# lofcz/Infidex

Hardware: AMD Instinct MI355X
Metric: queries/sec, 10M-doc corpus, top-k=20 (whole hot path, index resident in HBM) (higher is better)
Workload: dtype f32; 1 GPU; BASELINE config 4: 10000000 docs, vocab 1000000, 1 field(s), 1000-query batches, 2-3-word queries 30% fuzzed, depth 500, top-20; docs=10000000, batch=1000, top_k=20, coverage_depth=500, sessions_in_flight=4, parallelism=single GPU

## Files before the change

infidex_amd/csrc/infidex_hip.hip:

```cpp
#include <type_traits>
#include <cstring>
#include <hip/hip_runtime.h>
#include <stdint.h>
#include <string.h>
#include <stdio.h>
#include <string>
#include <vector>
#include <unordered_map>
#include <algorithm>
#include <map>
#include <mutex>
#include <chrono>
#include <thread>
#include <dlfcn.h>
#include <rccl/rccl.h>
#include "../../include/infidex_hip.h"
#include "unicode_tables.h"

#define WAVE 64
#define FILT_MAXCOL 64

static thread_local std::string g_err;
static int32_t fail(int32_t code, const char* fmt, const char* a = "") {
    char buf[512]; snprintf(buf, sizeof buf, fmt, a); g_err = buf; return code;
// ... 91 lines not shown
    uint64_t a = lo, b = hi;
    while (a < b) { uint64_t m = (a + b) >> 1; if ((int64_t)(packed ? (int32_t)((uint32_t)postDoc[m] >> 8) : postDoc[m]) < target) a = m + 1; else b = m; }
    skipTbl[(uint64_t)s * per + r] = (uint32_t)(a - lo);
}

__global__ void k_doc_norm(const float* docLen, float* norm, int n, float bDivAvg) {
    int i = blockIdx.x * blockDim.x + threadIdx.x;
    if (i >= n) return;
    const float k1 = 1.2f, minDl = 1.f - 0.75f;
    float t1 = bDivAvg * docLen[i];
    float t2 = minDl + t1;
    norm[i] = k1 * t2;
}

struct DevTerm {
    uint64_t begin, end;
    float idf;
    uint32_t skip;
    uint8_t role, rank, isVirtual, pad;
    uint16_t refIdx, pad2;
};
struct DevQuery {
    uint32_t termOff, numTerms;
    int32_t mode, prefixSet, depth, nAnd;
    uint32_t refOff, numRef;
};
struct SelRule {
    int32_t mode;
    int32_t cutoffRank;
    uint32_t classMask;
    int32_t depth;
    uint32_t total;
    uint32_t pad;
};

template <class Tp> __device__ __forceinline__ Tp rfl(Tp v) { return v; }
__device__ __forceinline__ int rfl_i(int v) { return __builtin_amdgcn_readfirstlane(v); }
__device__ __forceinline__ uint64_t rfl_u64(uint64_t v) {
    uint32_t lo = __builtin_amdgcn_readfirstlane((uint32_t)v), hi = __builtin_amdgcn_readfirstlane((uint32_t)(v >> 32));
    return ((uint64_t)hi << 32) | lo;
}

__device__ __forceinline__ int32_t post_doc(int32_t v, int packed) { return packed ? (int32_t)((uint32_t)v >> 8) : v; }
__device__ __forceinline__ uint64_t lower_bound_post(const int32_t* a, uint64_t lo, uint64_t hi, int32_t target, int packed) {
    while (lo < hi) { uint64_t m = (lo + hi) >> 1; if (post_doc(a[m], packed) < target) lo = m + 1; else hi = m; }
    return lo;
}
__device__ __forceinline__ uint64_t lower_bound_i32(const int32_t* a, uint64_t lo, uint64_t hi, int32_t target) {
    while (lo < hi) { uint64_t m = (lo + hi) >> 1; if (a[m] < target) lo = m + 1; else hi = m; }
    return lo;
}

#include "stage1.hip.inc"
#include "stage1_sparse.hip.inc"
#include "exact1.hip.inc"
#include "exact3.hip.inc"
#include "exactsh.hip.inc"
#include "stage2.hip.inc"

__host__ __device__ static inline SelRule make_rule0(const infx_query& Q, const uint32_t* c) {
    SelRule r{}; r.mode = Q.mode; r.depth = Q.depth; r.cutoffRank = 127; r.classMask = 0xFFFFFFFFu;
    const long k = Q.depth;
    if (Q.mode == INFX_MODE_AND) {
        unsigned long long t0 = 0, t1 = 0;
        for (int i = 0; i < 16; i++) { if (i & 1) t0 += c[i]; if (i & 2) t1 += c[i]; }
        if ((long)t0 >= k * 2) { r.classMask = 1; return r; }
        unsigned long long g = t0; uint32_t gmask = 1;
        if (Q.n_and >= 3 && (long)t0 < k * 3) { g = t1; gmask = 2 | 1; }
        if ((long)g < k * 5) {
            if (Q.df_s1 <= 0) { r.classMask = gmask; return r; }
            if ((long)Q.df_s1 >= k * 10 || Q.df_s2 <= 0) { r.classMask = 4 | gmask; return r; }
            r.classMask = 4 | 8 | gmask; return r;
        }
        r.classMask = gmask; return r;
    }
    if (Q.mode == INFX_MODE_DISJ) {
        int nElig = Q.n_and; bool hasSel = false; long local = 0; int cutoff = -1;
        int nRanks = 0; for (int i = 127; i >= 0; i--) if (c[i]) { nRanks = i + 1; break; }
        int totalRanks = nRanks > Q.df_s1 ? nRanks : Q.df_s1;
        for (int i = 0; i < totalRanks; i++) {
            bool lowq = i >= nElig;
            if (totalRanks > 1 && lowq && hasSel) continue;
            cutoff = i; local += c[i];
            if (!lowq && local > 0) hasSel = true;
            if (local >= k * 100) break;
        }
        r.cutoffRank = cutoff; return r;
    }
    return r;
}

__host__ __device__ static inline SelRule make_rule(const infx_query& Q, const uint32_t* c) {
    SelRule r = make_rule0(Q, c);
    unsigned long long tot = 0;
    if (Q.mode == INFX_MODE_AND) { for (int i = 0; i < 16; i++) if (i & r.classMask) tot += c[i]; }
    else if (Q.mode == INFX_MODE_DISJ) { for (int i = 0; i <= r.cutoffRank && i < 128; i++) tot += c[i]; tot += 128;  }
    else tot = c[1];
    r.total = (uint32_t)(tot < 0xFFFFFFFFull ? tot : 0xFFFFFFFFull); r.pad = 0;
    return r;
}

#include "fused.hip.inc"
#include "lookup.hip.inc"
#include "filter.hip.inc"
#include "browse.hip.inc"
#include "facets_filtered.hip.inc"
// ... 304 lines not shown
    if (!bytes) return INFX_OK;
    if (!is_device_ptr(src)) return up(s, dst, src, bytes);
    HIPCHK(hipMemcpyAsync(dst, src, bytes, hipMemcpyDeviceToDevice, s->st)); s->unsynced = true;
    return INFX_OK;
}
static int32_t downx(infx_stream* s, void* dst, const void* srcDev, size_t bytes) {
    if (!bytes) return INFX_OK;
    if (!is_device_ptr(dst)) return down(s, dst, srcDev, bytes);
    HIPCHK(hipMemcpyAsync(dst, srcDev, bytes, hipMemcpyDeviceToDevice, s->st)); s->unsynced = true;
    return INFX_OK;
}
struct PlanStream {
    infx_stream* s; bool on;
    explicit PlanStream(infx_stream* x) : s(x), on(x->stPlan != nullptr) { if (on) s->st = s->stPlan; }
    int32_t leave() {
        if (!on) return INFX_OK;
        on = false; s->st = s->stMain;
        HIPCHK(hipEventRecord(s->evPlan, s->stPlan));
        HIPCHK(hipStreamWaitEvent(s->stMain, s->evPlan, 0));
        return INFX_OK;
    }
    ~PlanStream() { if (on) s->st = s->stMain; }
};
#define UPX(dst, src, n) do { int32_t rc_ = upx(s, (dst), (src), (n)); if (rc_) return rc_; } while (0)
#define DOWNX(dst, src, n) do { int32_t rc_ = downx(s, (dst), (src), (n)); if (rc_) return rc_; } while (0)
#define UP(dst, src, n) do { int32_t rc_ = up(s, (dst), (src), (n)); if (rc_) return rc_; } while (0)
#define DOWN(dst, src, n) do { int32_t rc_ = down(s, (dst), (src), (n)); if (rc_) return rc_; } while (0)
#define SYNC() do { int32_t rc_ = stream_sync(s); if (rc_) return rc_; } while (0)
static int32_t table_upload(infx_stream* s, const ProgTable& T, void** buf, size_t* cap) {
    const size_t total = T.blob_bytes();
    { int32_t rc_ = grow(s, buf, cap, total); if (rc_) return rc_; }
    std::vector<uint8_t> H(total, 0);
    T.put_blob(H.data(), (const char*)*buf);
    return up(s, *buf, H.data(), total);
}
#define COLS_COVER_CORPUS "a column holds fewer rows than the corpus has documents%s"
#define COLS_COVER_COUNTED "a column holds fewer rows than the counted documents%s"
static int32_t columns_cover(const infx_index* ix, int64_t n, const char* msg, int col = -1) {
    for (int c = std::max(col, 0); c < (col < 0 ? FILT_MAXCOL : col + 1); c++)
        if (ix->colCodes[c] && (uint64_t)ix->colDocs[c] < (uint64_t)std::max<int64_t>(n, 0)) return fail(INFX_EINVAL, msg);
    return INFX_OK;
}
static DevColumns dev_columns(const infx_index* ix) { DevColumns cols; for (int c = 0; c < FILT_MAXCOL; c++) cols.codes[c] = ix->colCodes[c]; return cols; }
static hipError_t lds_limit(const void* fn, int device, size_t lds) {
    if (lds <= 64 * 1024) return hipSuccess;
    static std::mutex mu; static std::map<std::pair<int, const void*>, size_t> mark;
    std::lock_guard<std::mutex> lk(mu);
    size_t& hw = mark[{device, fn}];
    if (lds > hw) { const hipError_t e = hipFuncSetAttribute(fn, hipFuncAttributeMaxDynamicSharedMemorySize, (int)lds); if (e != hipSuccess) return e; hw = lds; }
    return hipSuccess;
}

template <int R> static void launch_union(infx_stream* s, uint32_t nv, const uint32_t* dBeg, const uint32_t* dEnd, const int32_t* dMembers, uint32_t* dRangeCount,
                                            const unsigned long long* dBase, int32_t* outDocs) {
    uint64_t blocks = (uint64_t)nv * s->ix->d.nRanges;
    k_union<R><<<dim3((unsigned)blocks), dim3(WAVE), 0, s->st>>>(dev_index(s), dBeg, dEnd, dMembers, nv, dRangeCount, dBase, outDocs);
}
static void launch_union_any(infx_stream* s, uint32_t nv, const uint32_t* dBeg, const uint32_t* dEnd, const int32_t* dMembers, uint32_t* dRangeCount,
                             const unsigned long long* dBase, int32_t* outDocs) {
    switch (s->ix->d.R) {
        case 512: launch_union<512>(s, nv, dBeg, dEnd, dMembers, dRangeCount, dBase, outDocs); break;
        case 1024: launch_union<1024>(s, nv, dBeg, dEnd, dMembers, dRangeCount, dBase, outDocs); break;
        case 2048: launch_union<2048>(s, nv, dBeg, dEnd, dMembers, dRangeCount, dBase, outDocs); break;
        case 4096: launch_union<4096>(s, nv, dBeg, dEnd, dMembers, dRangeCount, dBase, outDocs); break;
        case 8192: launch_union<8192>(s, nv, dBeg, dEnd, dMembers, dRangeCount, dBase, outDocs); break;
        default: launch_union<16384>(s, nv, dBeg, dEnd, dMembers, dRangeCount, dBase, outDocs); break;
    }
}
static bool exact_enabled(const infx_index* ix) { static const bool v = [] { const char* e = getenv("INFX_EXACT"); return !(e && e[0] == '0'); }(); return v && !(ix->cfg.flags & INFX_CFG_NO_EXACT_REPLAY); }
static Arena make_arena(infx_stream* s) {
    return Arena{s->arDoc, s->arScore, s->arCls, s->arMask, s->arExc, (const unsigned long long*)s->dBlockOut, (uint32_t*)s->dBlockOutHi,
                 (uint32_t*)s->dCounts, s->dOverflow, (unsigned long long*)s->dQBytes, (uint32_t*)((unsigned long long*)s->dQBytes + s->lastNqAlloc), (uint2*)s->dDir, s->maskWords};
}
static int acc_stripe() { static const int v = [] { const char* e = getenv("INFX_ACC_STRIPE"); int x = e ? atoi(e) : 0; return (x >= 1 && x <= 64) ? x : 4; }(); return v; }
template <int R> static bool acc_lds_layout_ok() {
    static const bool ok = [] {
        hipFuncAttributes a1{}, a2{}, a4{};
        if (hipFuncGetAttributes(&a1, (const void*)k_accumulate<R, 1>) != hipSuccess || hipFuncGetAttributes(&a2, (const void*)k_accumulate<R, 2>) != hipSuccess ||
            hipFuncGetAttributes(&a4, (const void*)k_accumulate<R, 4>) != hipSuccess) return false;
        return a1.sharedSizeBytes == 0 && a2.sharedSizeBytes == 0 && a4.sharedSizeBytes == 0;
    }();
    return ok;
}
static int acc_sparse_t() { static const int v = [] { const char* e = getenv("INFX_ACC_SPARSE_T"); const int x = e ? atoi(e) : 96; return std::max(0, std::min(4096, x)); }(); return v; }
template <int R> static void launch_acc(infx_stream* s, uint32_t nq, Arena ar, int maxT, int useGrp, int maxRef) {
    (void)maxRef;
    if (!acc_lds_layout_ok<R>()) { s->accLayoutBad = true; return; }
    static const int dbgSkip = [] { const char* e = getenv("INFX_ACC_SKIP"); return e ? atoi(e) : 0; }();
    const int sparseT = s->ix->hPostOff.empty() || s->ix->hPostOff.back() + 4 <= 0xFFFFFFF0ull ? acc_sparse_t() : 0;
    const int stripe = sparseT > 0 ? std::max(1, std::min(4, 65536 / R)) : acc_stripe();
    const int nStripes = (s->ix->d.nRanges + stripe - 1) / stripe;
    const uint64_t blocks = (uint64_t)nq * 8u * ((nStripes + 7) / 8);
    const uint8_t* dense = nullptr;
    if (sparseT > 0) {
        if (grow(s, &s->dDense, &s->capDense, (size_t)nq * nStripes)) { s->accLayoutBad = true; return; }
        hipMemsetAsync(s->dDense, 0, (size_t)nq * nStripes, s->st);
        const size_t sw = (size_t)stripe * (R / 32);
        const int maxTl = (std::min(64, std::max(1, maxT)) + 3) & ~3;
        static const int dbgS = [] { const char* e = getenv("INFX_ACCS_SKIP"); return e ? atoi(e) : 0; }();
        const size_t ldsS = (sw + 64 + 4) * 4 + INFX_NCLASS * 4 + WAVE * 2 + WAVE * 12 + (size_t)WAVE * maxTl + (size_t)64 * maxTl;
#define ACCS_LAUNCH(MW_) k_accumulate_sparse<R, MW_><<<dim3((unsigned)blocks), dim3(WAVE), ldsS, s->st>>>(dev_index(s), (const DevQuery*)s->dQueries, (const DevTerm*)s->dTerms, (const int32_t*)s->dExtra, \
            (const int32_t*)s->dUDocs, (const uint32_t*)s->dURange, nq, ar, stripe, useGrp, (uint8_t*)s->dDense, (uint32_t)sparseT, nStripes, maxTl, dbgS)
        if (ar.maskWords == 4) ACCS_LAUNCH(4); else if (ar.maskWords == 2) ACCS_LAUNCH(2); else ACCS_LAUNCH(1);
#undef ACCS_LAUNCH
        dense = (const uint8_t*)s->dDense;
    }
    const size_t lds = (size_t)R + 128 + ((size_t)(R / 32) + 2) * 4 + INFX_NCLASS * 4 + ACC_CAP_DEFAULT * 2;
#define ACC_LAUNCH(MW_) k_accumulate<R, MW_><<<dim3((unsigned)blocks), dim3(WAVE), lds, s->st>>>(dev_index(s), (const DevQuery*)s->dQueries, (const DevTerm*)s->dTerms, (const int32_t*)s->dExtra, \
        (const int32_t*)s->dUDocs, (const uint32_t*)s->dURange, nq, ar, maxT, stripe, useGrp, dbgSkip, (unsigned long long*)s->dStats, dense, nStripes, \
        s->nAccHeavy != 0xFFFFFFFFu ? (const uint32_t*)s->dAccOrder : nullptr, s->nAccHeavy != 0xFFFFFFFFu ? s->nAccHeavy : 0u)
    if (ar.maskWords == 4) ACC_LAUNCH(4); else if (ar.maskWords == 2) ACC_LAUNCH(2); else ACC_LAUNCH(1);
#undef ACC_LAUNCH
    if (dbgSkip & 8) { unsigned long long h[4] = {0, 0, 0, 0}; hipStreamSynchronize(s->st); hipMemcpy(h, s->dStats, 32, hipMemcpyDeviceToHost); hipMemset(s->dStats, 0, 32);
        fprintf(stderr, "[infx] k_accumulate stats: %llu ranges with candidates (%llu blocks), %.2f rounds/range, %.1f candidates/range\n", h[0], (unsigned long long)blocks, h[0] ? (double)h[1] / h[0] : 0.0, h[0] ? (double)h[2] / h[0] : 0.0); }
}

static const uint32_t* select_order(infx_stream* s, uint32_t nq) {
    static const bool off = [] { const char* e = getenv("INFX_SELECT_LPT"); return e && e[0] == '0'; }();
    if (off || nq < 64 || nq > SEL_ORDER_MAX) return nullptr;
// ... 1867 lines not shown
    std::vector<FusedMeta> metas(nq);
    if (s1) DOWN(s1, s->dFS1, (size_t)nq * depth * sizeof(infx_hit));
    if (cands) DOWN(cands, s->dCovC, ncand * sizeof(infx_cov_cand));
    if (outs) DOWN(outs, s->dCovO, ncand * sizeof(infx_cov_out));
    if (feat) DOWN(feat, s->dCovF, ncand * INFX_NFEAT * 4);
    DOWN(metas.data(), s->dFMeta, (size_t)nq * sizeof(FusedMeta));
    SYNC();
    for (uint32_t i = 0; i < nq; i++) {
        if (s1_counts) s1_counts[i] = metas[i].s1Count;
        if (cand_counts) cand_counts[i] = metas[i].candCount;
        if (run_cov) run_cov[i] = metas[i].runCov | (metas[i].wmAny << 1);
        if (idx01) { idx01[2 * i] = metas[i].idx0; idx01[2 * i + 1] = metas[i].idx1; }
    }
    return INFX_OK;
}

int32_t infx_last_fused_stats(infx_stream* s, uint64_t* s1_rows, uint64_t* stage2_rows, uint64_t* stage2_text_bytes) {
    if (!s) return fail(INFX_EINVAL, "null argument%s");
    if (s1_rows) *s1_rows = s->fusedS1; if (stage2_rows) *stage2_rows = s->fusedCands; if (stage2_text_bytes) *stage2_text_bytes = s->fusedTextBytes;
    return INFX_OK;
}

int32_t infx_last_fused_timings(infx_stream* s, float* ms5) {
    if (!s || !ms5) return fail(INFX_EINVAL, "null argument%s");
    if (s->timedFused) {
        hipEventElapsedTime(&s->msFused[0], s->evA0, s->evA1); hipEventElapsedTime(&s->msFused[1], s->evS0, s->evS1);
        hipEventElapsedTime(&s->msFused[2], s->evP0, s->evP1); hipEventElapsedTime(&s->msFused[3], s->evC0, s->evC1);
        hipEventElapsedTime(&s->msFused[4], s->evF0, s->evF1);
    }
    for (int i = 0; i < 5; i++) ms5[i] = s->msFused[i];
    return INFX_OK;
}

int32_t infx_last_timings(infx_stream* s, float* a, float* b, float* c) {
    if (!s) return fail(INFX_EINVAL, "null argument%s");
    if (s->timedAcc) hipEventElapsedTime(&s->msAcc, s->evA0, s->evA1);
    if (s->timedSel) hipEventElapsedTime(&s->msSel, s->evS0, s->evS1);
    if (s->timedCov) hipEventElapsedTime(&s->msCov, s->evC0, s->evC1);
    if (a) *a = s->msAcc; if (b) *b = s->msSel; if (c) *c = s->msCov;
    return INFX_OK;
}
static int32_t union_build_impl(infx_stream* s, uint32_t nv, const uint32_t* member_offs, const int32_t* members, uint32_t* counts_out,
                                const int32_t* word_of, uint32_t nwords, const uint32_t* word_offs, const uint16_t* chars, uint32_t cap,
                                int32_t* ld1_members_out, uint32_t* ld1_counts_out, uint32_t* ld1_status_out) {
    s->unionCount.clear(); s->unionBase.assign(1, 0);
    if (nv == 0) return INFX_OK;
    infx_index* ix = s->ix;
    if (!ix->havePostings || !ix->haveDocs) return fail(INFX_EINVAL, "index not uploaded%s");
    if (nwords && !ix->haveTrie) return fail(INFX_EINVAL, "infx_upload_term_trie has not been called%s");
    HIPCHK(enter_device(ix->cfg.device));
    { int32_t rc_ = pin_reset(s); if (rc_) return rc_; }
    PlanStream plan(s);
    const int nR = ix->d.nRanges;
    if ((uint64_t)nv * nR > 0x7FFFFFFFull) return fail(INFX_ECAPACITY, "nv * nRanges exceeds the grid limit%s");
    const uint32_t nm = member_offs[nv];
    for (uint32_t i = 0; i < nm; i++) if (members[i] < 0 || members[i] >= ix->d.T) return fail(INFX_EINVAL, "member term id out of range%s");
    if ((uint64_t)nm + (uint64_t)nwords * cap > 0xFFFFFFF0ull) return fail(INFX_ECAPACITY, "too many union members in one batch%s");
    std::vector<uint32_t> be((size_t)nv * 2); std::vector<int32_t> uow(nwords, -1);
    for (uint32_t v = 0; v < nv; v++) {
        const int32_t w = word_of ? word_of[v] : -1;
        if (w >= 0) { if ((uint32_t)w >= nwords || uow[w] >= 0 || member_offs[v + 1] != member_offs[v]) return fail(INFX_EINVAL, "bad word reference of a union%s"); uow[w] = (int32_t)v; be[v] = nm + (uint32_t)w * cap; be[nv + v] = be[v]; }
        else { be[v] = member_offs[v]; be[nv + v] = member_offs[v + 1]; }
    }
    GROW(s->dUOffs, s->capUOffs, ((size_t)nv * 2 + 2) * 4);
    GROW(s->dUMem, s->capUMem, std::max<size_t>(1, (size_t)nm + (size_t)nwords * cap) * 4);
    GROW(s->dUCnt, s->capUCnt, (size_t)nv * 4);
    GROW(s->dURange, s->capURange, (size_t)nv * (nR + 1) * 4);
    GROW(s->dUBase, s->capUBase, ((size_t)nv + 1) * 8);
    UP(s->dUOffs, be.data(), be.size() * 4);
    UP(s->dUMem, members, (size_t)nm * 4);
    uint32_t* dBeg = (uint32_t*)s->dUOffs; uint32_t* dEnd = dBeg + nv;
    uint32_t *dCnt = nullptr, *dSt = nullptr;
    if (nwords) {
        const size_t nch = word_offs[nwords];
        GROW(s->dLWordOff, s->capLWordOff, ((size_t)nwords * 2 + 2) * 4);
        GROW(s->dLChars, s->capLChars, std::max<size_t>(1, nch) * 2);
        GROW(s->dLCount, s->capLCount, (size_t)nwords * 8);
        UP(s->dLWordOff, word_offs, ((size_t)nwords + 1) * 4);
        UP((uint32_t*)s->dLWordOff + nwords + 1, uow.data(), (size_t)nwords * 4);
        UP(s->dLChars, chars, nch * 2);
        dCnt = (uint32_t*)s->dLCount; dSt = dCnt + nwords;
        k_ld1<<<nwords, WAVE, 0, s->st>>>(*ix->lk, (const uint32_t*)s->dLWordOff, (const uint16_t*)s->dLChars, nwords, cap, (int32_t*)s->dUMem + nm, dCnt, dSt,
                                          dEnd, (const int32_t*)((uint32_t*)s->dLWordOff + nwords + 1), nm);
        HIPCHK(hipGetLastError());
    }
    launch_union_any(s, nv, dBeg, dEnd, (const int32_t*)s->dUMem, (uint32_t*)s->dURange, nullptr, nullptr);
    k_union_scan<<<nv, 256, 0, s->st>>>((uint32_t*)s->dURange, nR, (uint32_t*)s->dUCnt);
    HIPCHK(hipGetLastError());
    DOWN(counts_out, s->dUCnt, (size_t)nv * 4);
    if (nwords) { DOWN(ld1_counts_out, dCnt, (size_t)nwords * 4); DOWN(ld1_status_out, dSt, (size_t)nwords * 4); DOWN(ld1_members_out, (const int32_t*)s->dUMem + nm, (size_t)nwords * cap * 4); }
    SYNC();
    s->unionCount.assign(counts_out, counts_out + nv);
    s->unionBase.assign((size_t)nv + 1, 0);
    for (uint32_t v = 0; v < nv; v++) s->unionBase[v + 1] = s->unionBase[v] + ((counts_out[v] + 3u) & ~3u);
    GROW(s->dUDocs, s->capUDocs, ((size_t)s->unionBase[nv] + 4) * 4);
    HIPCHK(hipMemsetAsync(s->dUDocs, 0x7F, ((size_t)s->unionBase[nv] + 4) * 4, s->st));
    UP(s->dUBase, s->unionBase.data(), ((size_t)nv + 1) * 8);
    launch_union_any(s, nv, dBeg, dEnd, (const int32_t*)s->dUMem, (uint32_t*)s->dURange, (const unsigned long long*)s->dUBase, (int32_t*)s->dUDocs);
    HIPCHK(hipGetLastError());
    return plan.leave();
}
int32_t infx_union_build(infx_stream* s, uint32_t nv, const uint32_t* member_offs, const int32_t* members, uint32_t* counts_out) {
    if (!s || (nv && (!member_offs || !counts_out || (member_offs[nv] && !members)))) return fail(INFX_EINVAL, "null argument%s");
    return union_build_impl(s, nv, member_offs, members, counts_out, nullptr, 0, nullptr, nullptr, 1, nullptr, nullptr, nullptr);
}
int32_t infx_union_build_ld1(infx_stream* s, uint32_t nv, const uint32_t* member_offs, const int32_t* members, const int32_t* word_of,
                             uint32_t nwords, const uint32_t* word_offs, const uint16_t* chars, uint32_t cap,
                             uint32_t* counts_out, int32_t* ld1_members_out, uint32_t* ld1_counts_out, uint32_t* ld1_status_out) {
    if (!s || (nv && (!member_offs || !counts_out || (member_offs[nv] && !members))) || (nwords && (!word_of || !word_offs || !ld1_members_out || !ld1_counts_out || !ld1_status_out || (word_offs[nwords] && !chars))) || cap == 0)
        return fail(INFX_EINVAL, "null argument%s");
    return union_build_impl(s, nv, member_offs, members, counts_out, nwords ? word_of : nullptr, nwords, word_offs, chars, cap, ld1_members_out, ld1_counts_out, ld1_status_out);
}
int32_t infx_last_replay_stats(infx_stream* s, float* ms, uint32_t* why3) {
    if (!s) return fail(INFX_EINVAL, "null argument%s");
    if (s->timedReplay) { hipEventElapsedTime(&s->msReplay, s->evX0, s->evX1); s->timedReplay = false; }
    if (ms) *ms = s->msReplay;
    if (why3) { why3[0] = s->lastFlagWhy[0]; why3[1] = s->lastFlagWhy[1]; why3[2] = s->lastFlagWhy[2]; }
    return INFX_OK;
}
int32_t infx_last_replay_breakdown(infx_stream* s, float* ms4) {
    if (!s || !ms4) return fail(INFX_EINVAL, "null argument%s");
    if (s->timedReplayParts) {
        hipEventElapsedTime(&s->msReplayParts[0], s->evX0, s->evXa); hipEventElapsedTime(&s->msReplayParts[1], s->evXa, s->evXb);
        hipEventElapsedTime(&s->msReplayParts[2], s->evXb, s->evXc); hipEventElapsedTime(&s->msReplayParts[3], s->evXc, s->evX1);
        s->timedReplayParts = false;
    }
    for (int i = 0; i < 4; i++) ms4[i] = s->msReplayParts[i];
    return INFX_OK;
}
int32_t infx_last_exact_replays(infx_stream* s, uint32_t* n) {
    if (!s || !n) return fail(INFX_EINVAL, "null argument%s");
    *n = s->lastExact2[0] + s->lastExact2[1]; return INFX_OK;
}
int32_t infx_last_exact_fallbacks(infx_stream* s, uint32_t* n) {
    if (!s || !n) return fail(INFX_EINVAL, "null argument%s");
    *n = s->lastExact2[1]; return INFX_OK;
}
int32_t infx_last_candidates(infx_stream* s, uint64_t* n) {
    if (!s || !n) return fail(INFX_EINVAL, "null argument%s");
    *n = s->lastCandTotal; return INFX_OK;
}
int32_t infx_last_alg_bytes(infx_stream* s, uint64_t* bytes) {
    if (!s || !bytes) return fail(INFX_EINVAL, "null argument%s");
    *bytes = s->lastAlgBytes; return INFX_OK;
}


int32_t infx_upload_column(infx_index* ix, uint32_t col, uint32_t total_docs, const uint32_t* codes, uint32_t num_values) {
    if (!ix || col >= FILT_MAXCOL || (total_docs && !codes)) return fail(INFX_EINVAL, "bad column arguments%s");
    HIPCHK(enter_device(ix->cfg.device));
    if (ix->haveDocs && (uint64_t)total_docs < (uint64_t)ix->d.docBase + (uint64_t)ix->d.N) return fail(INFX_EINVAL, "a column needs one code per GLOBAL internal id covering this shard%s");
// ... 1442 lines not shown
```

infidex_amd/csrc/stage1.hip.inc:

```

#define F_LOWEST 0x100
#define F_S1 0x200
#define F_S2 0x400
#define CLS_HOLE 0xFF

struct Arena {
    int32_t* doc; float* score; uint8_t* cls;
    unsigned long long* mask;
    uint32_t* exc;
    const unsigned long long* qBase;
    uint32_t* qCursor;
    uint32_t* counts;
    uint32_t* overflow;
    unsigned long long* qBytes;
    uint32_t* qMax;
    uint2* dir;
    int maskWords;
};

#define ACC_WPS 4
#define ACC_PF 2
#define ACC_G 2
#define ACC_CAP_DEFAULT (64 * ACC_G)

// ... 322 lines not shown
            if (s < nslot && sc > 0.f) {
                if (mode == INFX_MODE_AND) {
                    if (f & (F_S1 | F_S2)) {
                        emit = true;
                        const int c2 = (int)(f & 0xFF);
                        const bool t1 = c2 == nAnd - 1;
                        const bool t0b = t1 && (f & F_LOWEST);
                        cls = (uint8_t)((t0b ? 1 : 0) | ((t1 && nAnd >= 3) ? 2 : 0) | ((f & F_S1) ? 4 : 0) | ((f & F_S2) ? 8 : 0));
                        atomicAdd(&sHist[cls], 1u);
                    }
                } else if (mode == INFX_MODE_DISJ) {
                    if (f != 0) {
                        emit = true;
                        cls = (uint8_t)((f - 1) & 0x7F);
                        bool pre = false;
                        if (psLen) {
                            int32_t d = base + l;
                            uint64_t p = lower_bound_i32(ix.psDocs, psBase, psBase + psLen, d);
                            pre = p < psBase + psLen && ix.psDocs[p] == d;
                        }
                        if (pre) cls |= 0x80; else atomicAdd(&sHist[cls], 1u);
                    }
                } else { emit = true; cls = 1; atomicAdd(&sHist[1], 1u); }
            }
            const unsigned long long m = __ballot(emit);
            if (emit) {
                const unsigned long long pos = outBase + written + __popcll(m & ((1ull << lane) - 1));
                ar.doc[pos] = ix.docBase + base + l;
                const float stored = (del && del[ix.docBase + base + l]) ? 0.f : sc;
                ar.score[pos] = stored; myMax = max(myMax, __float_as_uint(stored));
                ar.cls[pos] = cls;
                if (ar.maskWords) {
#pragma unroll
                    for (int w = 0; w < MW; w++) ar.mask[pos * (unsigned long long)MW + w] = cMask[g][w];
                    ar.exc[pos] = cExc[g];
                }
            }
            written += (uint32_t)__popcll(m);
        }
    }
    if (!haveOff || dropped) continue;
    if (lane == 0) { ar.dir[(unsigned long long)q * ix.nRanges + r] = make_uint2(chunkOff, written); myBytes += (unsigned long long)written * 12ull; }
    for (uint32_t i = written + lane; i < ncand; i += WAVE) { ar.cls[outBase + i] = CLS_HOLE; ar.score[outBase + i] = 0.f; }
    }
    for (int i = lane; i < INFX_NCLASS; i += WAVE) { uint32_t c = sHist[i]; if (c) atomicAdd(&ar.counts[(uint64_t)q * INFX_NCLASS + i], c); }
#pragma unroll
    for (int d = 32; d > 0; d >>= 1) myBytes += __shfl_down(myBytes, d);
    if (lane == 0 && myBytes) atomicAdd(&ar.qBytes[q], myBytes);
#pragma unroll
    for (int d = 32; d > 0; d >>= 1) myMax = max(myMax, (uint32_t)__shfl_down((int)myMax, d));
    if (lane == 0 && myMax) atomicMax(&ar.qMax[q], myMax);
}

template <int R>
__global__ __launch_bounds__(WAVE) void k_union(DevIndex ix, const uint32_t* __restrict__ memberBeg, const uint32_t* __restrict__ memberEnd, const int32_t* __restrict__ members,
                                                 uint32_t nv, uint32_t* __restrict__ rangeCount, const unsigned long long* __restrict__ unionBase,
                                                 int32_t* __restrict__ outDocs) {
    constexpr int W = R / 32;
    constexpr int WPL = (W + WAVE - 1) / WAVE;
    __shared__ uint32_t sBits[W];
    __shared__ unsigned long long sBase[WAVE];
    __shared__ uint32_t sLen[WAVE];
    const int lane = threadIdx.x;
    const uint32_t v = blockIdx.x % nv; const int r = (int)(blockIdx.x / nv);
    const int32_t base = r * R, rend = min(base + R, ix.N);
    if (outDocs) { if (r + 1 <= ix.nRanges && rangeCount[(uint64_t)v * (ix.nRanges + 1) + r] == rangeCount[(uint64_t)v * (ix.nRanges + 1) + r + 1]) return; }
    for (int i = lane; i < W; i += WAVE) sBits[i] = 0;
    const uint32_t mb = memberBeg[v], me = memberEnd[v];
    bool any = false;
    for (uint32_t m0 = mb; m0 < me; m0 += WAVE) {
        uint32_t len = 0; unsigned long long b0 = 0;
        if (m0 + lane < me) {
            const int32_t t = members[m0 + lane];
            const uint64_t tb = ix.postOff[t], te = ix.postOff[t + 1];
            const uint32_t sk = ix.skipIdx[t];
            uint32_t lo, hi;
            if (sk != 0xFFFFFFFFu) { lo = ix.skipTbl[sk + r]; hi = ix.skipTbl[sk + r + 1]; }
            else { lo = (uint32_t)(lower_bound_post(ix.postDoc, tb, te, base, ix.packed) - tb); hi = (uint32_t)(lower_bound_post(ix.postDoc, tb + lo, te, rend, ix.packed) - tb); }
            len = hi - lo; b0 = tb + lo;
        }
        sBase[lane] = b0; sLen[lane] = len;
        const int nm = (int)min((uint32_t)WAVE, me - m0);
        for (int k = 0; k < nm; k++) {
            const uint32_t L = sLen[k]; const unsigned long long bb = sBase[k];
            if (L) any = true;
            for (uint32_t i = lane; i < L; i += WAVE) { int l = post_doc(ix.postDoc[bb + i], ix.packed) - base; atomicOr(&sBits[l >> 5], 1u << (l & 31)); }
        }
    }
    if (!outDocs) {
        uint32_t c = 0;
        if (any) for (int i = lane; i < W; i += WAVE) c += __popc(sBits[i]);
#pragma unroll
        for (int d = 32; d > 0; d >>= 1) c += __shfl_down(c, d);
        if (lane == 0) rangeCount[(uint64_t)v * (ix.nRanges + 1) + r] = c;
        return;
    }
    if (!any) return;
    uint32_t myBits[WPL]; uint32_t cnt = 0;
#pragma unroll
    for (int j = 0; j < WPL; j++) { int wi = lane * WPL + j; myBits[j] = wi < W ? sBits[wi] : 0u; cnt += __popc(myBits[j]); }
    uint32_t incl = cnt;
#pragma unroll
    for (int d = 1; d < WAVE; d <<= 1) { uint32_t x = __shfl_up(incl, d); if (lane >= d) incl += x; }
    unsigned long long o = unionBase[v] + rangeCount[(uint64_t)v * (ix.nRanges + 1) + r] + (incl - cnt);
#pragma unroll
    for (int j = 0; j < WPL; j++) {
        uint32_t bits = myBits[j]; const int wi = lane * WPL + j;
        while (bits) { int bpos = __ffs(bits) - 1; bits &= bits - 1; outDocs[o++] = base + wi * 32 + bpos; }
    }
}
__global__ __launch_bounds__(256) void k_union_scan(uint32_t* __restrict__ rangeCount, int nRanges, uint32_t* __restrict__ totals) {
    __shared__ uint32_t sPart[256];
    const uint32_t v = blockIdx.x; const int tid = threadIdx.x;
    uint32_t* rc = rangeCount + (uint64_t)v * (nRanges + 1);
    const int per = (nRanges + 255) / 256;
    const int b0 = tid * per, b1 = min(nRanges, b0 + per);
    uint32_t s = 0; for (int i = b0; i < b1; i++) s += rc[i];
    sPart[tid] = s; __syncthreads();
    if (tid == 0) { uint32_t run = 0; for (int i = 0; i < 256; i++) { uint32_t x = sPart[i]; sPart[i] = run; run += x; } totals[v] = run; rc[nRanges] = run; }
    __syncthreads();
    uint32_t run = sPart[tid];
    for (int i = b0; i < b1; i++) { uint32_t x = rc[i]; rc[i] = run; run += x; }
}

#define SEL_THREADS 1024
#define SEL_WAVES (SEL_THREADS / WAVE)
#define SEL_CAP 2048
#define SEL_AMBIG_REL 1e-5f

__device__ __forceinline__ bool sel_pass(const SelRule& rule, uint8_t c) {
    if (rule.mode == INFX_MODE_AND) return (c & rule.classMask) != 0;
    if (rule.mode == INFX_MODE_DISJ) return (int)(c & 0x7F) <= rule.cutoffRank;
    return true;
}
__device__ __forceinline__ unsigned long long sel_key(const Arena& ar, uint64_t i) {
    return ((unsigned long long)__float_as_uint(ar.score[i]) << 32) | (0xFFFFFFFFu - (uint32_t)ar.doc[i]);
}

#ifndef SEL_U
#define SEL_U 8
#endif
template <class F> __device__ __forceinline__ void sel_sweep(const Arena& ar, const SelRule& rule, uint64_t qb, uint32_t qn, int tid, F&& f) {
    for (uint32_t i0 = tid; i0 < qn; i0 += SEL_U * SEL_THREADS) {
        uint8_t c[SEL_U]; uint32_t sb[SEL_U];
#pragma unroll
        for (int u = 0; u < SEL_U; u++) { const uint32_t i = i0 + u * SEL_THREADS; c[u] = i < qn ? ar.cls[qb + i] : (uint8_t)CLS_HOLE; sb[u] = i < qn ? __float_as_uint(ar.score[qb + i]) : 0u; }
#pragma unroll
        for (int u = 0; u < SEL_U; u++) if (sb[u] && sel_pass(rule, c[u])) f(sb[u], i0 + u * SEL_THREADS);
    }
}

#define SEL_ORDER_MAX 4096
__global__ __launch_bounds__(1024) void k_select_order(const uint32_t* __restrict__ qCursor, uint32_t nq, uint32_t* __restrict__ order) {
    __shared__ unsigned long long sK[SEL_ORDER_MAX];
    const uint32_t tid = threadIdx.x;
    uint32_t m = 2; while (m < nq) m <<= 1;
    for (uint32_t i = tid; i < m; i += 1024) sK[i] = i < nq ? (((unsigned long long)qCursor[i] << 32) | (0xFFFFFFFFu - i)) : 0ull;
    __syncthreads();
    for (uint32_t k = 2; k <= m; k <<= 1)
        for (uint32_t j = k >> 1; j > 0; j >>= 1) {
            for (uint32_t t = tid; t < (m >> 1); t += 1024) {
                const uint32_t a = ((t & ~(j - 1)) << 1) | (t & (j - 1)), b = a | j;
                const unsigned long long va = sK[a], vb = sK[b];
                const bool desc = (a & k) == 0;
                if (desc ? (va < vb) : (va > vb)) { sK[a] = vb; sK[b] = va; }
            }
            __syncthreads();
        }
    for (uint32_t i = tid; i < nq; i += 1024) order[i] = 0xFFFFFFFFu - (uint32_t)sK[i];
}
#define SELG_MAX 256
#define SELG_SHIFT2 16
#define SELG_PARTS 32
#define SELG_PART_MIN 16384
struct SelGiant { uint32_t* hist; uint32_t* count; uint32_t* left; uint32_t* mode; uint32_t* cut; uint32_t* shift; unsigned long long* keys; uint32_t minRows; };
__device__ __forceinline__ bool selg_part(const Arena& ar, const SelRule* __restrict__ rules, const uint32_t* __restrict__ order, uint32_t nq, const SelGiant& G,
                                          int& q, uint64_t& qb, uint32_t& r0, uint32_t& rn) {
// ... 302 lines not shown
```

Baseline: 90630 queries/s.

## Union posting lists per 32K-doc slab with balanced vectorized posting streaming

Replaces the per-range union kernel (one wave per variant×range) with a slab kernel in which each block covers 32768 docs, i.e. many ranges. Member postings are streamed as aligned int4 loads, with work balanced across threads through a prefix scan and a binary search over the member offsets. The host memset of the output union-doc buffer is dropped and the kernel writes the padding instead. The scan kernel now uses wave shuffles instead of a serial loop. The aim is to cut block count, per-range skip-lookup overhead and the memset pass, at the cost of larger LDS bitmaps and extra work in empty slabs. An optional stats counter, off by default, is also added.

```diff
diff --git a/infidex_amd/csrc/infidex_hip.hip b/infidex_amd/csrc/infidex_hip.hip
--- a/infidex_amd/csrc/infidex_hip.hip
+++ b/infidex_amd/csrc/infidex_hip.hip
@@ -167,6 +167,7 @@
 }
 
 #include "stage1.hip.inc"
+#include "union.hip.inc"
 #include "stage1_sparse.hip.inc"
 #include "exact1.hip.inc"
 #include "exact3.hip.inc"
@@ -577,19 +578,19 @@
 }
 
 template <int R> static void launch_union(infx_stream* s, uint32_t nv, const uint32_t* dBeg, const uint32_t* dEnd, const int32_t* dMembers, uint32_t* dRangeCount,
-                                            const unsigned long long* dBase, int32_t* outDocs) {
-    uint64_t blocks = (uint64_t)nv * s->ix->d.nRanges;
-    k_union<R><<<dim3((unsigned)blocks), dim3(WAVE), 0, s->st>>>(dev_index(s), dBeg, dEnd, dMembers, nv, dRangeCount, dBase, outDocs);
+                                            const unsigned long long* dBase, int32_t* outDocs, unsigned long long* stats) {
+    const uint64_t blocks = (uint64_t)nv * (uint64_t)us_n_slabs(s->ix->d.nRanges, R);
+    k_union_slab<R><<<dim3((unsigned)blocks), dim3(UNION_THREADS), 0, s->st>>>(dev_index(s), dBeg, dEnd, dMembers, nv, dRangeCount, dBase, outDocs, stats);
 }
 static void launch_union_any(infx_stream* s, uint32_t nv, const uint32_t* dBeg, const uint32_t* dEnd, const int32_t* dMembers, uint32_t* dRangeCount,
-                             const unsigned long long* dBase, int32_t* outDocs) {
+                             const unsigned long long* dBase, int32_t* outDocs, unsigned long long* stats) {
     switch (s->ix->d.R) {
-        case 512: launch_union<512>(s, nv, dBeg, dEnd, dMembers, dRangeCount, dBase, outDocs); break;
-        case 1024: launch_union<1024>(s, nv, dBeg, dEnd, dMembers, dRangeCount, dBase, outDocs); break;
-        case 2048: launch_union<2048>(s, nv, dBeg, dEnd, dMembers, dRangeCount, dBase, outDocs); break;
-        case 4096: launch_union<4096>(s, nv, dBeg, dEnd, dMembers, dRangeCount, dBase, outDocs); break;
-        case 8192: launch_union<8192>(s, nv, dBeg, dEnd, dMembers, dRangeCount, dBase, outDocs); break;
-        default: launch_union<16384>(s, nv, dBeg, dEnd, dMembers, dRangeCount, dBase, outDocs); break;
+        case 512: launch_union<512>(s, nv, dBeg, dEnd, dMembers, dRangeCount, dBase, outDocs, stats); break;
+        case 1024: launch_union<1024>(s, nv, dBeg, dEnd, dMembers, dRangeCount, dBase, outDocs, stats); break;
+        case 2048: launch_union<2048>(s, nv, dBeg, dEnd, dMembers, dRangeCount, dBase, outDocs, stats); break;
+        case 4096: launch_union<4096>(s, nv, dBeg, dEnd, dMembers, dRangeCount, dBase, outDocs, stats); break;
+        case 8192: launch_union<8192>(s, nv, dBeg, dEnd, dMembers, dRangeCount, dBase, outDocs, stats); break;
+        default: launch_union<16384>(s, nv, dBeg, dEnd, dMembers, dRangeCount, dBase, outDocs, stats); break;
     }
 }
 static bool exact_enabled(const infx_index* ix) { static const bool v = [] { const char* e = getenv("INFX_EXACT"); return !(e && e[0] == '0'); }(); return v && !(ix->cfg.flags & INFX_CFG_NO_EXACT_REPLAY); }
@@ -2563,7 +2564,7 @@
     { int32_t rc_ = pin_reset(s); if (rc_) return rc_; }
     PlanStream plan(s);
     const int nR = ix->d.nRanges;
-    if ((uint64_t)nv * nR > 0x7FFFFFFFull) return fail(INFX_ECAPACITY, "nv * nRanges exceeds the grid limit%s");
+    if ((uint64_t)nv * (uint64_t)us_n_slabs(nR, ix->d.R) > 0x7FFFFFFFull) return fail(INFX_ECAPACITY, "nv * slabs exceeds the grid limit%s");
     const uint32_t nm = member_offs[nv];
     for (uint32_t i = 0; i < nm; i++) if (members[i] < 0 || members[i] >= ix->d.T) return fail(INFX_EINVAL, "member term id out of range%s");
     if ((uint64_t)nm + (uint64_t)nwords * cap > 0xFFFFFFF0ull) return fail(INFX_ECAPACITY, "too many union members in one batch%s");
@@ -2595,19 +2596,29 @@
                                           dEnd, (const int32_t*)((uint32_t*)s->dLWordOff + nwords + 1), nm);
         HIPCHK(hipGetLastError());
     }
-    launch_union_any(s, nv, dBeg, dEnd, (const int32_t*)s->dUMem, (uint32_t*)s->dURange, nullptr, nullptr);
+    static const bool wantStats = [] { const char* e = getenv("INFX_UNION_STATS"); return e && e[0] == '1'; }();
+    unsigned long long* dStats = nullptr;
+    if (wantStats) { HIPCHK(hipMalloc((void**)&dStats, 16)); HIPCHK(hipMemsetAsync(dStats, 0, 16, s->st)); }
+    launch_union_any(s, nv, dBeg, dEnd, (const int32_t*)s->dUMem, (uint32_t*)s->dURange, nullptr, nullptr, dStats);
     k_union_scan<<<nv, 256, 0, s->st>>>((uint32_t*)s->dURange, nR, (uint32_t*)s->dUCnt);
     HIPCHK(hipGetLastError());
     DOWN(counts_out, s->dUCnt, (size_t)nv * 4);
     if (nwords) { DOWN(ld1_counts_out, dCnt, (size_t)nwords * 4); DOWN(ld1_status_out, dSt, (size_t)nwords * 4); DOWN(ld1_members_out, (const int32_t*)s->dUMem + nm, (size_t)nwords * cap * 4); }
+    unsigned long long hStats[2] = {0, 0};
+    if (dStats) DOWN(hStats, dStats, 16);
     SYNC();
+    if (dStats) {
+        unsigned long long docs = 0; for (uint32_t v = 0; v < nv; v++) docs += counts_out[v];
+        fprintf(stderr, "INFX_UNION_STATS nv %u members %u ranges %d slabs %d nonempty_slabs %llu of %llu postings_streamed %llu union_docs %llu\n", nv, nm, nR,
+                us_n_slabs(nR, ix->d.R), hStats[0], (unsigned long long)nv * us_n_slabs(nR, ix->d.R), hStats[1], docs);
+        hipFree(dStats);
+    }
     s->unionCount.assign(counts_out, counts_out + nv);
     s->unionBase.assign((size_t)nv + 1, 0);
     for (uint32_t v = 0; v < nv; v++) s->unionBase[v + 1] = s->unionBase[v] + ((counts_out[v] + 3u) & ~3u);
     GROW(s->dUDocs, s->capUDocs, ((size_t)s->unionBase[nv] + 4) * 4);
-    HIPCHK(hipMemsetAsync(s->dUDocs, 0x7F, ((size_t)s->unionBase[nv] + 4) * 4, s->st));
     UP(s->dUBase, s->unionBase.data(), ((size_t)nv + 1) * 8);
-    launch_union_any(s, nv, dBeg, dEnd, (const int32_t*)s->dUMem, (uint32_t*)s->dURange, (const unsigned long long*)s->dUBase, (int32_t*)s->dUDocs);
+    launch_union_any(s, nv, dBeg, dEnd, (const int32_t*)s->dUMem, (uint32_t*)s->dURange, (const unsigned long long*)s->dUBase, (int32_t*)s->dUDocs, nullptr);
     HIPCHK(hipGetLastError());
     return plan.leave();
 }
diff --git a/infidex_amd/csrc/stage1.hip.inc b/infidex_amd/csrc/stage1.hip.inc
--- a/infidex_amd/csrc/stage1.hip.inc
+++ b/infidex_amd/csrc/stage1.hip.inc
@@ -398,77 +398,6 @@
     if (lane == 0 && myMax) atomicMax(&ar.qMax[q], myMax);
 }
 
-template <int R>
-__global__ __launch_bounds__(WAVE) void k_union(DevIndex ix, const uint32_t* __restrict__ memberBeg, const uint32_t* __restrict__ memberEnd, const int32_t* __restrict__ members,
-                                                 uint32_t nv, uint32_t* __restrict__ rangeCount, const unsigned long long* __restrict__ unionBase,
-                                                 int32_t* __restrict__ outDocs) {
-    constexpr int W = R / 32;
-    constexpr int WPL = (W + WAVE - 1) / WAVE;
-    __shared__ uint32_t sBits[W];
-    __shared__ unsigned long long sBase[WAVE];
-    __shared__ uint32_t sLen[WAVE];
-    const int lane = threadIdx.x;
-    const uint32_t v = blockIdx.x % nv; const int r = (int)(blockIdx.x / nv);
-    const int32_t base = r * R, rend = min(base + R, ix.N);
-    if (outDocs) { if (r + 1 <= ix.nRanges && rangeCount[(uint64_t)v * (ix.nRanges + 1) + r] == rangeCount[(uint64_t)v * (ix.nRanges + 1) + r + 1]) return; }
-    for (int i = lane; i < W; i += WAVE) sBits[i] = 0;
-    const uint32_t mb = memberBeg[v], me = memberEnd[v];
-    bool any = false;
-    for (uint32_t m0 = mb; m0 < me; m0 += WAVE) {
-        uint32_t len = 0; unsigned long long b0 = 0;
-        if (m0 + lane < me) {
-            const int32_t t = members[m0 + lane];
-            const uint64_t tb = ix.postOff[t], te = ix.postOff[t + 1];
-            const uint32_t sk = ix.skipIdx[t];
-            uint32_t lo, hi;
-            if (sk != 0xFFFFFFFFu) { lo = ix.skipTbl[sk + r]; hi = ix.skipTbl[sk + r + 1]; }
-            else { lo = (uint32_t)(lower_bound_post(ix.postDoc, tb, te, base, ix.packed) - tb); hi = (uint32_t)(lower_bound_post(ix.postDoc, tb + lo, te, rend, ix.packed) - tb); }
-            len = hi - lo; b0 = tb + lo;
-        }
-        sBase[lane] = b0; sLen[lane] = len;
-        const int nm = (int)min((uint32_t)WAVE, me - m0);
-        for (int k = 0; k < nm; k++) {
-            const uint32_t L = sLen[k]; const unsigned long long bb = sBase[k];
-            if (L) any = true;
-            for (uint32_t i = lane; i < L; i += WAVE) { int l = post_doc(ix.postDoc[bb + i], ix.packed) - base; atomicOr(&sBits[l >> 5], 1u << (l & 31)); }
-        }
-    }
-    if (!outDocs) {
-        uint32_t c = 0;
-        if (any) for (int i = lane; i < W; i += WAVE) c += __popc(sBits[i]);
-#pragma unroll
-        for (int d = 32; d > 0; d >>= 1) c += __shfl_down(c, d);
-        if (lane == 0) rangeCount[(uint64_t)v * (ix.nRanges + 1) + r] = c;
-        return;
-    }
-    if (!any) return;
-    uint32_t myBits[WPL]; uint32_t cnt = 0;
-#pragma unroll
-    for (int j = 0; j < WPL; j++) { int wi = lane * WPL + j; myBits[j] = wi < W ? sBits[wi] : 0u; cnt += __popc(myBits[j]); }
-    uint32_t incl = cnt;
-#pragma unroll
-    for (int d = 1; d < WAVE; d <<= 1) { uint32_t x = __shfl_up(incl, d); if (lane >= d) incl += x; }
-    unsigned long long o = unionBase[v] + rangeCount[(uint64_t)v * (ix.nRanges + 1) + r] + (incl - cnt);
-#pragma unroll
-    for (int j = 0; j < WPL; j++) {
-        uint32_t bits = myBits[j]; const int wi = lane * WPL + j;
-        while (bits) { int bpos = __ffs(bits) - 1; bits &= bits - 1; outDocs[o++] = base + wi * 32 + bpos; }
-    }
-}
-__global__ __launch_bounds__(256) void k_union_scan(uint32_t* __restrict__ rangeCount, int nRanges, uint32_t* __restrict__ totals) {
-    __shared__ uint32_t sPart[256];
-    const uint32_t v = blockIdx.x; const int tid = threadIdx.x;
-    uint32_t* rc = rangeCount + (uint64_t)v * (nRanges + 1);
-    const int per = (nRanges + 255) / 256;
-    const int b0 = tid * per, b1 = min(nRanges, b0 + per);
-    uint32_t s = 0; for (int i = b0; i < b1; i++) s += rc[i];
-    sPart[tid] = s; __syncthreads();
-    if (tid == 0) { uint32_t run = 0; for (int i = 0; i < 256; i++) { uint32_t x = sPart[i]; sPart[i] = run; run += x; } totals[v] = run; rc[nRanges] = run; }
-    __syncthreads();
-    uint32_t run = sPart[tid];
-    for (int i = b0; i < b1; i++) { uint32_t x = rc[i]; rc[i] = run; run += x; }
-}
-
 #define SEL_THREADS 1024
 #define SEL_WAVES (SEL_THREADS / WAVE)
 #define SEL_CAP 2048
diff --git a/infidex_amd/csrc/union.hip.inc b/infidex_amd/csrc/union.hip.inc
--- /dev/null
+++ b/infidex_amd/csrc/union.hip.inc
@@ -0,0 +1,159 @@
+#include "union_slabs.h"
+#ifndef UNION_THREADS
+#define UNION_THREADS 64
+#endif
+#define UNION_WAVES (UNION_THREADS / WAVE)
+#define US_WPW (US_SLAB_WORDS / UNION_WAVES)
+static_assert(UNION_THREADS % WAVE == 0 && US_SLAB_WORDS % (UNION_WAVES * WAVE) == 0 && US_SLAB_WORDS % 4 == 0, "a wave owns whole steps of 64 words, the clear stores 16 bytes");
+
+__device__ __forceinline__ uint32_t us_scan(uint32_t x, uint32_t* sWave, int lane, int wave, uint32_t& total) {
+    uint32_t incl = x;
+#pragma unroll
+    for (int d = 1; d < WAVE; d <<= 1) { const uint32_t y = __shfl_up(incl, d); if (lane >= d) incl += y; }
+    if (lane == WAVE - 1) sWave[wave] = incl;
+    __syncthreads();
+    total = 0;
+#pragma unroll
+    for (int w = 0; w < UNION_WAVES; w++) { const uint32_t t = sWave[w]; if (w < wave) incl += t; total += t; }
+    __syncthreads();
+    return incl;
+}
+
+template <int R>
+__global__ __launch_bounds__(UNION_THREADS) void k_union_slab(DevIndex ix, const uint32_t* __restrict__ memberBeg, const uint32_t* __restrict__ memberEnd,
+                                                             const int32_t* __restrict__ members, uint32_t nv, uint32_t* __restrict__ rangeCount,
+                                                             const unsigned long long* __restrict__ unionBase, int32_t* __restrict__ outDocs,
+                                                             unsigned long long* __restrict__ stats) {
+    constexpr int W = R / 32;
+    static_assert(US_SLAB_DOCS % R == 0, "a slab holds whole ranges");
+    static_assert(US_WPW % W == 0, "a wave holds whole ranges");
+    __shared__ __attribute__((aligned(16))) uint32_t sBits[US_SLAB_WORDS];
+    __shared__ unsigned long long sBase[UNION_THREADS];
+    __shared__ uint32_t sEnd[UNION_THREADS];
+    __shared__ uint32_t sWave[UNION_WAVES];
+    const int tid = threadIdx.x, lane = tid & (WAVE - 1), wave = tid / WAVE;
+    const uint32_t v = blockIdx.x % nv; const int slab = (int)(blockIdx.x / nv);
+    const int r0 = us_first_range(slab, R), r1 = us_end_range(slab, ix.nRanges, R);
+    const int32_t base = r0 * R, send = min(r1 * R, ix.N);
+    const uint32_t span = (uint32_t)(send - base);
+    uint32_t* rc = rangeCount + (uint64_t)v * (ix.nRanges + 1);
+    if (outDocs) {
+        if (r1 == ix.nRanges) {
+            const unsigned long long ub = unionBase[v];
+            const uint32_t total = rc[ix.nRanges];
+            if (total + tid < ((total + 3u) & ~3u)) outDocs[ub + total + tid] = 0x7F7F7F7F;
+            if (v == nv - 1 && tid < 4) outDocs[unionBase[nv] + tid] = 0x7F7F7F7F;
+        }
+        if (rc[r0] == rc[r1]) return;
+    }
+    const uint32_t mb = memberBeg[v], me = memberEnd[v];
+    bool clear = false;
+    for (uint32_t m0 = mb; m0 < me; m0 += UNION_THREADS) {
+        uint32_t len = 0, ng = 0; unsigned long long a0 = 0;
+        if (m0 + tid < me) {
+            const int32_t t = members[m0 + tid];
+            const uint64_t tb = ix.postOff[t], te = ix.postOff[t + 1];
+            const uint32_t sk = ix.skipIdx[t];
+            uint32_t lo, hi;
+            if (sk != 0xFFFFFFFFu) { lo = ix.skipTbl[sk + r0]; hi = ix.skipTbl[sk + r1]; }
+            else { lo = (uint32_t)(lower_bound_post(ix.postDoc, tb, te, base, ix.packed) - tb); hi = (uint32_t)(lower_bound_post(ix.postDoc, tb + lo, te, send, ix.packed) - tb); }
+            len = hi - lo;
+            const uint32_t mis = (uint32_t)(tb + lo) & 3u;
+            a0 = tb + lo - mis;
+            if (len) ng = (len + mis + 3u) >> 2;
+        }
+        uint32_t total;
+        const uint32_t incl = us_scan(ng, sWave, lane, wave, total);
+        if (!total) continue;
+        sBase[tid] = a0; sEnd[tid] = incl;
+        if (stats && len && !outDocs) atomicAdd(&stats[1], (unsigned long long)len);
+        if (!clear) {
+            for (int i = tid * 4; i < US_SLAB_WORDS; i += UNION_THREADS * 4) *(uint4*)(sBits + i) = make_uint4(0, 0, 0, 0);
+            clear = true;
+        }
+        __syncthreads();
+        const int nm = (int)min((uint32_t)UNION_THREADS, me - m0);
+        for (uint32_t g = (uint32_t)tid; g < total; g += UNION_THREADS) {
+            int k = 0;
+            for (int s = UNION_THREADS >> 1; s; s >>= 1) if (k + s <= nm && sEnd[k + s - 1] <= g) k += s;
+            const uint32_t first = k ? sEnd[k - 1] : 0u;
+            const int4 p = ld4((gint4p)(uintptr_t)(ix.postDoc + sBase[k]), g - first);
+            const uint32_t l0 = (uint32_t)(post_doc(p.x, ix.packed) - base), l1 = (uint32_t)(post_doc(p.y, ix.packed) - base);
+            const uint32_t l2 = (uint32_t)(post_doc(p.z, ix.packed) - base), l3 = (uint32_t)(post_doc(p.w, ix.packed) - base);
+            if (l0 < span) atomicOr(&sBits[l0 >> 5], 1u << (l0 & 31));
+            if (l1 < span) atomicOr(&sBits[l1 >> 5], 1u << (l1 & 31));
+            if (l2 < span) atomicOr(&sBits[l2 >> 5], 1u << (l2 & 31));
+            if (l3 < span) atomicOr(&sBits[l3 >> 5], 1u << (l3 & 31));
+        }
+    }
+    if (!clear) {
+        if (!outDocs) for (int r = r0 + tid; r < r1; r += UNION_THREADS) rc[r] = 0;
+        return;
+    }
+    __syncthreads();
+    if (stats && tid == 0 && !outDocs) atomicAdd(&stats[0], 1ull);
+    const uint32_t* mine = sBits + wave * US_WPW;
+    if (!outDocs) {
+        if constexpr (W >= WAVE) {
+            for (int j = 0; j < US_WPW / W; j++) {
+                const int r = r0 + wave * (US_WPW / W) + j;
+                if (r >= r1) break;
+                uint32_t c = 0;
+#pragma unroll
+                for (int s = 0; s < W / WAVE; s++) c += __popc(mine[j * W + s * WAVE + lane]);
+#pragma unroll
+                for (int d = 1; d < WAVE; d <<= 1) c += __shfl_xor(c, d);
+                if (lane == 0) rc[r] = c;
+            }
+        } else {
+            for (int s = 0; s < US_WPW / WAVE; s++) {
+                uint32_t c = __popc(mine[s * WAVE + lane]);
+#pragma unroll
+                for (int d = 1; d < W; d <<= 1) c += __shfl_xor(c, d);
+                const int r = r0 + (wave * US_WPW + s * WAVE + lane) / W;
+                if (lane % W == 0 && r < r1) rc[r] = c;
+            }
+        }
+        return;
+    }
+    uint32_t before = 0;
+    if constexpr (UNION_WAVES > 1) {
+        uint32_t c = 0;
+        for (int s = 0; s < US_WPW / WAVE; s++) c += __popc(mine[s * WAVE + lane]);
+#pragma unroll
+        for (int d = 1; d < WAVE; d <<= 1) c += __shfl_xor(c, d);
+        if (lane == 0) sWave[wave] = c;
+        __syncthreads();
+        for (int w = 0; w < wave; w++) before += sWave[w];
+    }
+    unsigned long long o = unionBase[v] + rc[r0] + before;
+    for (int s = 0; s < US_WPW / WAVE; s++) {
+        uint32_t bits = mine[s * WAVE + lane];
+        const uint32_t cnt = __popc(bits);
+        if (!__ballot(cnt != 0)) continue;
+        uint32_t incl = cnt;
+#pragma unroll
+        for (int d = 1; d < WAVE; d <<= 1) { const uint32_t y = __shfl_up(incl, d); if (lane >= d) incl += y; }
+        unsigned long long oo = o + (incl - cnt);
+        const int32_t d0 = base + (wave * US_WPW + s * WAVE + lane) * 32;
+        while (bits) { const int bpos = __ffs(bits) - 1; bits &= bits - 1; outDocs[oo++] = d0 + bpos; }
+        o += rdl_u(incl, WAVE - 1);
+    }
+}
+__global__ __launch_bounds__(256) void k_union_scan(uint32_t* __restrict__ rangeCount, int nRanges, uint32_t* __restrict__ totals) {
+    __shared__ uint32_t sWave[256 / WAVE];
+    const uint32_t v = blockIdx.x; const int tid = threadIdx.x, lane = tid & (WAVE - 1), wave = tid / WAVE;
+    uint32_t* rc = rangeCount + (uint64_t)v * (nRanges + 1);
+    const int per = (nRanges + 255) / 256;
+    const int b0 = tid * per, b1 = min(nRanges, b0 + per);
+    uint32_t s = 0; for (int i = b0; i < b1; i++) s += rc[i];
+    uint32_t incl = s;
+#pragma unroll
+    for (int d = 1; d < WAVE; d <<= 1) { const uint32_t x = __shfl_up(incl, d); if (lane >= d) incl += x; }
+    if (lane == WAVE - 1) sWave[wave] = incl;
+    __syncthreads();
+    uint32_t run = incl - s;
+    for (int w = 0; w < wave; w++) run += sWave[w];
+    if (tid == 255) { totals[v] = run + s; rc[nRanges] = run + s; }
+    for (int i = b0; i < b1; i++) { const uint32_t x = rc[i]; rc[i] = run; run += x; }
+}
diff --git a/infidex_amd/csrc/union_slabs.h b/infidex_amd/csrc/union_slabs.h
--- /dev/null
+++ b/infidex_amd/csrc/union_slabs.h
@@ -0,0 +1,14 @@
+#pragma once
+#include <stdint.h>
+#ifndef US_FN
+#define US_FN __host__ __device__ __forceinline__
+#endif
+#ifndef US_SLAB_DOCS
+#define US_SLAB_DOCS 32768
+#endif
+#define US_SLAB_WORDS (US_SLAB_DOCS / 32)
+
+US_FN constexpr int us_slab_ranges(int R) { return US_SLAB_DOCS / R; }
+US_FN constexpr int us_n_slabs(int nRanges, int R) { return (nRanges + us_slab_ranges(R) - 1) / us_slab_ranges(R); }
+US_FN constexpr int us_first_range(int slab, int R) { return slab * us_slab_ranges(R); }
+US_FN constexpr int us_end_range(int slab, int nRanges, int R) { return (slab + 1) * us_slab_ranges(R) < nRanges ? (slab + 1) * us_slab_ranges(R) : nRanges; }
```

Result: slower. 89140 queries/s (-1.6%).
